# rohitsinghlab/SAME

Measured on AMD Instinct MI355X. Metric: cell-pairs/sec on 100k×100k cost build + edge-cross sweep; % HBM roofline, higher is better.
Workload: dtype f64

## Files before the change

### include/same_hip_diag.h

```cpp
#ifndef SAME_HIP_DIAG_H
#define SAME_HIP_DIAG_H

#include "same_hip.h"

#ifdef __cplusplus
extern "C" {
#endif

enum { SAME_STAT_LAUNCHES = 0, SAME_STAT_FILLS = 1, SAME_STAT_COPIES = 2, SAME_STAT_WAITS = 3, SAME_STAT_GREEDY_READBACKS = 4, SAME_STAT_COUNT = 5 };
int same_ctx_stat(same_ctx *ctx, int which, int64_t *out);


int same_timer_start(same_ctx *ctx);
int same_timer_stop(same_ctx *ctx, float *out_ms);
int same_timer_mark(same_ctx *ctx);
int same_timer_read(same_ctx *ctx, float *out_ms);

int same_ctx_pci_bus_id(same_ctx *ctx, char *out, size_t out_len);
int same_dev_mem_info(same_ctx *ctx, int64_t *out_free, int64_t *out_total);

#define SAME_SPREAD_INFO_LEN 14
int same_dev_alloc_spread(same_ctx *ctx, size_t bytes, void **out_dptr, int64_t *out_info);

#define SAME_Q32_MAX_TYPES 32
int same_quantize_u32_dev(same_ctx *ctx, const double *dsrc, int64_t n, double offset, double scale,
                          uint32_t *ddst);
int same_dense_cost_q32_dev(same_ctx *ctx, const uint32_t *dAq, const uint32_t *dRq, const double *dA,
                            const double *dR, int T, const double *daxy, const double *drxy, int64_t n_r,
                            int64_t row_begin, int64_t row_end, double w, double inv_scale,
                            double rel_tol, double *dout, int64_t ld);

int same_comm_gather_time(same_ctx *ctx, float *out_ms, int64_t *out_send_bytes);

#ifdef __cplusplus
}
#endif
#endif
```

### same_amd/_lib.py

```python
import ctypes
import os
import sys
import threading

import numpy as np

_HERE = os.path.dirname(os.path.abspath(__file__))
LIB_PATH = os.environ.get("SAME_HIP_LIB") or os.path.join(_HERE, "libsame_hip.so")

c_i64 = ctypes.c_int64
c_int = ctypes.c_int
c_dbl = ctypes.c_double
c_flt = ctypes.c_float
c_vp = ctypes.c_void_p
c_sz = ctypes.c_size_t

UNIQUE_ID_BYTES = 128
ABI_VERSION = 9
DT_U8, DT_I32, DT_U64, DT_F64 = 0, 1, 2, 3
OP_SUM, OP_MAX, OP_MIN = 0, 1, 2
SPREAD_INFO_LEN = 14
MAX_KNN = 448
ALIGN_MAX_KNN = 64
ALIGN_MATCH, ALIGN_DECIDED = 1, 2
MAX_TYPES = 4096

_PROTOTYPES = {
    "same_abi_version": [],
    "same_device_count": [ctypes.POINTER(c_int)],
    "same_ctx_create": [c_int, ctypes.POINTER(c_vp)],
    "same_ctx_destroy": [c_vp],
    "same_ctx_sync": [c_vp],
    "same_strerror": [c_int],
    "same_last_error": [c_vp],
    "same_ctx_info": [c_vp, ctypes.c_char_p, c_sz, ctypes.POINTER(c_int), ctypes.POINTER(c_i64)],
    "same_ctx_pci_bus_id": [c_vp, ctypes.c_char_p, c_sz],
    "same_ctx_stat": [c_vp, c_int, ctypes.POINTER(c_i64)],
    "same_dev_alloc": [c_vp, c_sz, ctypes.POINTER(c_vp)],
    "same_dev_free": [c_vp, c_vp],
    "same_dev_alloc_spread": [c_vp, c_sz, ctypes.POINTER(c_vp), ctypes.POINTER(c_i64)],
    "same_h2d": [c_vp, c_vp, c_vp, c_sz],
    "same_d2h": [c_vp, c_vp, c_vp, c_sz],
    "same_dev_memset": [c_vp, c_vp, c_int, c_sz],
    "same_d2d": [c_vp, c_vp, c_vp, c_sz],
    "same_dev_mem_info": [c_vp, ctypes.POINTER(c_i64), ctypes.POINTER(c_i64)],
    "same_ctx_release_scratch": [c_vp],
    "same_timer_start": [c_vp],
    "same_timer_stop": [c_vp, ctypes.POINTER(c_flt)],
    "same_timer_mark": [c_vp],
    "same_timer_read": [c_vp, ctypes.POINTER(c_flt)],
    "same_pair_cost_f64": [c_vp, c_vp, c_vp, c_i64, c_i64, c_int, c_vp, c_vp, c_vp, c_i64, c_dbl, c_vp],
    "same_pair_cost_f32": [c_vp, c_vp, c_vp, c_i64, c_i64, c_int, c_vp, c_vp, c_vp, c_i64, c_flt, c_vp],
    "same_dense_cost_f64_dev": [c_vp, c_vp, c_vp, c_int, c_vp, c_vp, c_i64, c_i64, c_i64, c_dbl, c_vp, c_i64],
    "same_dense_cost_f32_dev": [c_vp, c_vp, c_vp, c_int, c_vp, c_vp, c_i64, c_i64, c_i64, c_flt, c_vp, c_i64],
    "same_dense_cost_f64": [c_vp, c_vp, c_vp, c_i64, c_i64, c_int, c_vp, c_vp, c_i64, c_i64, c_dbl, c_vp, c_i64],
    "same_dense_cost_f32": [c_vp, c_vp, c_vp, c_i64, c_i64, c_int, c_vp, c_vp, c_i64, c_i64, c_flt, c_vp, c_i64],
    "same_quantize_u32_dev": [c_vp, c_vp, c_i64, c_dbl, c_dbl, c_vp],
    "same_dense_cost_q32_dev": [c_vp, c_vp, c_vp, c_vp, c_vp, c_int, c_vp, c_vp, c_i64, c_i64, c_i64, c_dbl, c_dbl, c_dbl, c_vp, c_i64],
    "same_knn_prune": [c_vp, c_vp, c_i64, c_vp, c_i64, c_i64, c_i64, c_dbl, c_int, c_vp, c_vp, c_vp],
    "same_knn_prune_dev": [c_vp, c_vp, c_vp, c_i64, c_i64, c_i64, c_dbl, c_int, c_vp, c_vp, c_vp],
    "same_knn_index_build": [c_vp, c_vp, c_i64, c_dbl, ctypes.POINTER(c_vp)],
    "same_knn_index_destroy": [c_vp],
    "same_knn_prune_indexed_dev": [c_vp, c_vp, c_vp, c_i64, c_i64, c_int, c_vp, c_vp, c_vp],
    "same_padded_cost_f64_dev": [c_vp, c_vp, c_vp, c_int, c_vp, c_vp, c_i64, c_i64, c_int, c_vp, c_dbl, c_vp],
    "same_padded_cost_f32_dev": [c_vp, c_vp, c_vp, c_int, c_vp, c_vp, c_i64, c_i64, c_int, c_vp, c_flt, c_vp],
    "same_tri_classify": [c_vp, c_vp, c_i64, c_vp, c_i64, c_dbl, c_int, c_dbl, c_vp, c_vp, c_vp, c_vp],
    "same_tri_sign_weight": [c_vp, c_vp, c_vp, c_i64, c_vp, c_i64, c_vp, c_vp],
    "same_sweep_bind": [c_vp, c_vp, c_i64, c_vp, c_vp, c_i64, c_i64, c_vp, c_i64, ctypes.POINTER(c_vp)],
    "same_sweep_unbind": [c_vp],
    "same_orient_sweep": [c_vp, c_vp, c_i64, ctypes.POINTER(c_i64), c_vp, ctypes.POINTER(c_i64), c_vp],
# ... 329 lines not shown
```

### same_amd/csrc/common.h

```cpp
#pragma once
#include <hip/hip_runtime.h>

#include <cstdint>
#include <cstdio>
#include <cstring>
#include <string>
#include <vector>

#include "same_hip_diag.h"

struct ncclComm;

enum Slot {
    SL_A = 0, SL_R, SL_AXY, SL_RXY, SL_PAIRS, SL_OUT0, SL_OUT1, SL_OUT2, SL_TRIS, SL_MATCH,
    SL_SIGN, SL_SIZE, SL_TYPE, SL_FLAG0, SL_FLAG1, SL_FLAG2, SL_COUNTS, SL_X, SL_MASK,
    SL_K_HIST, SL_K_RANK, SL_K_SXY, SL_K_SIDX, SL_K_BBOX, SL_K_START,
    SL_Q_START, SL_Q_RANK, SL_Q_SXY, SL_Q_SIDX,
    SL_COUNT
};

struct same_spread_alloc {
    char *va = nullptr;
    size_t bytes = 0;
    std::vector<void *> handles;
};
void same_spread_release(same_spread_alloc &a);

struct same_ctx {
    int device = -1;
    hipStream_t stream = nullptr;
    hipStream_t comm_stream = nullptr;
    hipEvent_t ev0 = nullptr, ev1 = nullptr;
    hipEvent_t ev_ready = nullptr, ev_gathered = nullptr;
    hipEvent_t ev_gather0 = nullptr;
    bool gather_open = false, gather_stamped = false, in_group = false;
    size_t gather_bytes = 0;
    void *slot[SL_COUNT] = {};
    size_t slot_bytes[SL_COUNT] = {};
    void *pinned = nullptr;
    size_t pinned_bytes = 0;
    std::string err;
    int cu_count = 0;
    ncclComm *comm = nullptr;
    int nranks = 1, rank = 0;
    std::vector<same_spread_alloc> spread;
    int64_t stats[SAME_STAT_COUNT] = {};
};

#define SAME_LAUNCH(ctx, kernel, grid, block, lds, ...)                                  \
    do {                                                                                 \
// ... 123 lines not shown
            csr[2 * (size_t)q] = (int32_t)i;
            csr[2 * (size_t)q + 1] = j;
            out->ccsr[(size_t)q] = costs[p];
        }
    return SAME_OK;
}

int same_pair_rowmin_core(same_ctx *ctx, const int32_t *dpairs, const double *dcosts, int64_t P, int64_t n_m, double *dout);
int same_greedy_core(same_ctx *ctx, const int32_t *dpairs, const double *dcosts, int64_t P, int64_t n_m, int64_t n_r,
                     const uint8_t *dprefer, int32_t *dmatch_pair, int *out_rounds);

constexpr int SAME_GREEDY_BATCH_MAX = 64;
struct same_greedy_state {
    uint8_t *alive = nullptr;
    uint8_t *used = nullptr;
    unsigned long long *key[2] = {nullptr, nullptr};
    unsigned *idx[2] = {nullptr, nullptr};
    unsigned long long *sel = nullptr;
    bool float_costs = false;
};
int same_greedy_rounds_core(same_ctx *ctx, const int32_t *dpairs, const double *dcosts, int64_t P, const unsigned long long *dP,
                            int64_t n_m, int64_t n_r, const same_greedy_state &st, int32_t *dmatch_pair, int first, int count);

constexpr int SAME_LAUNCH_WINDOWS = 8;
struct same_greedy_job {
    const int32_t *pairs = nullptr;
    const double *costs = nullptr;
    int64_t P = 0, n_m = 0, n_r = 0;
    same_greedy_state st;
    int32_t *match_pair = nullptr;
};
int same_greedy_rounds_batch_core(same_ctx *ctx, const same_greedy_job *jobs, int n_jobs, int first, int count);

int same_sort_u64_core(same_ctx *ctx, unsigned long long *dkey, int64_t n_pad);
int same_merge_dedup_core(same_ctx *ctx, const uint8_t *dviol, unsigned viol_mask, const int32_t *dwin, const int32_t *da, const int32_t *dr,
                          int64_t n, int32_t *dout, unsigned long long *dtotal);

struct same_knn_index;
struct same_knn_window_job {
    const int32_t *rows_m = nullptr;
    const unsigned long long *dn_m = nullptr;
    int64_t cap_m = 0;
    const int32_t *rows_r = nullptr;
    const unsigned long long *dn_r = nullptr;
    double box[4] = {0, 0, 0, 0};
    int32_t *idx = nullptr, *cnt = nullptr;
};
int same_knn_window_batch_core(same_ctx *ctx, const same_knn_index *ix, const double *dmov_xy, const same_knn_window_job *jobs, int n_jobs, int k);
struct same_cost_window_job {
    const int32_t *rows = nullptr;
    const unsigned long long *dn = nullptr;
    int64_t cap = 0;
    const int32_t *idx = nullptr;
    void *out = nullptr;
};
int same_padded_cost_window_batch_core(same_ctx *ctx, int cost_f32, const void *dA, const void *dR, int T, const void *daxy_c, const void *drxy_c,
                                       const same_cost_window_job *jobs, int n_jobs, int k, double w);
```

### same_amd/csrc/merge.hip

```cpp
#include <algorithm>

#include "common.h"
#include "scan.h"

namespace {

constexpr int SORT_BLOCK = 2048;

__global__ __launch_bounds__(256) void merge_key_kernel(const uint8_t *__restrict__ viol, unsigned viol_mask, const int32_t *__restrict__ window, int64_t n,
                                                          int64_t n_pad, unsigned long long *__restrict__ key) {
    const int64_t i = (int64_t)blockIdx.x * blockDim.x + threadIdx.x;
    if (i >= n_pad) return;
    key[i] = i < n ? ((unsigned long long)((viol[i] & viol_mask) ? 1 : 0) << 63) | ((unsigned long long)(uint32_t)window[i] << 32) | (unsigned long long)i
                   : ~0ull;
}

__global__ __launch_bounds__(256) void bitonic_global_kernel(unsigned long long *__restrict__ key, int64_t n_pad, int64_t j, int64_t k) {
    const int64_t t = (int64_t)blockIdx.x * blockDim.x + threadIdx.x;
    if (t >= n_pad / 2) return;
    const int64_t lo = ((t / j) * 2 * j) + (t % j), hi = lo + j;
    const bool up = (lo & k) == 0;
    const unsigned long long a = key[lo], b = key[hi];
    if ((a > b) == up) { key[lo] = b; key[hi] = a; }
}

__global__ __launch_bounds__(1024) void bitonic_lds_kernel(unsigned long long *__restrict__ key, int64_t k, int j_top) {
    __shared__ unsigned long long s[SORT_BLOCK];
    const int64_t base = (int64_t)blockIdx.x * SORT_BLOCK;
    s[threadIdx.x] = key[base + threadIdx.x];
    s[threadIdx.x + 1024] = key[base + threadIdx.x + 1024];
    __syncthreads();
    for (int j = j_top; j >= 1; j >>= 1) {
        const int t = threadIdx.x;
        const int lo = ((t / j) * 2 * j) + (t % j), hi = lo + j;
        const bool up = ((base + lo) & k) == 0;
        const unsigned long long a = s[lo], b = s[hi];
        if ((a > b) == up) { s[lo] = b; s[hi] = a; }
        __syncthreads();
    }
    key[base + threadIdx.x] = s[threadIdx.x];
    key[base + threadIdx.x + 1024] = s[threadIdx.x + 1024];
}

__global__ __launch_bounds__(1024) void bitonic_lds_head_kernel(unsigned long long *__restrict__ key) {
    __shared__ unsigned long long s[SORT_BLOCK];
    const int64_t base = (int64_t)blockIdx.x * SORT_BLOCK;
    s[threadIdx.x] = key[base + threadIdx.x];
    s[threadIdx.x + 1024] = key[base + threadIdx.x + 1024];
    __syncthreads();
    for (int k = 2; k <= SORT_BLOCK; k <<= 1)
        for (int j = k >> 1; j >= 1; j >>= 1) {
            const int t = threadIdx.x;
            const int lo = ((t / j) * 2 * j) + (t % j), hi = lo + j;
            const bool up = ((base + lo) & k) == 0;
            const unsigned long long a = s[lo], b = s[hi];
            if ((a > b) == up) { s[lo] = b; s[hi] = a; }
            __syncthreads();
        }
    key[base + threadIdx.x] = s[threadIdx.x];
    key[base + threadIdx.x + 1024] = s[threadIdx.x + 1024];
}

__device__ __forceinline__ uint64_t mix64(uint64_t x) {
    x ^= x >> 30; x *= 0xbf58476d1ce4e5b9ull;
    x ^= x >> 27; x *= 0x94d049bb133111ebull;
    return x ^ (x >> 31);
}

constexpr unsigned long long EMPTY = ~0ull;

__device__ __forceinline__ int64_t pair_slot(unsigned long long *__restrict__ tkey, int64_t mask, unsigned long long pair) {
    int64_t h = (int64_t)(mix64(pair) & (uint64_t)mask);
    for (;;) {
        const unsigned long long seen = atomicCAS(&tkey[h], EMPTY, pair);
        if (seen == EMPTY || seen == pair) return h;
        h = (h + 1) & mask;
    }
}

__global__ __launch_bounds__(256) void merge_first_kernel(const unsigned long long *__restrict__ key, int64_t n, const int32_t *__restrict__ a_code,
                                                            const int32_t *__restrict__ r_code, unsigned long long *__restrict__ tkey,
                                                            unsigned int *__restrict__ tfirst, int64_t mask) {
    const int64_t s = (int64_t)blockIdx.x * blockDim.x + threadIdx.x;
    if (s >= n) return;
    const uint32_t row = (uint32_t)key[s];
    const unsigned long long pair = ((unsigned long long)(uint32_t)a_code[row] << 32) | (uint32_t)r_code[row];
    atomicMin(&tfirst[pair_slot(tkey, mask, pair)], (unsigned int)s);
}

__global__ __launch_bounds__(scan::NT) void merge_compact_kernel(const unsigned long long *__restrict__ key, int64_t n, const int32_t *__restrict__ a_code,
                                                                  const int32_t *__restrict__ r_code, unsigned long long *__restrict__ tkey,
                                                                  const unsigned int *__restrict__ tfirst, int64_t mask,
                                                                  unsigned long long *__restrict__ status, int32_t *__restrict__ out_rows,
                                                                  unsigned long long *__restrict__ out_total) {
    __shared__ scan::Shared sh;
    auto keep_of = [&](int64_t q) -> bool {
        if (q >= n) return false;
        const uint32_t row = (uint32_t)key[q];
        const unsigned long long pair = ((unsigned long long)(uint32_t)a_code[row] << 32) | (uint32_t)r_code[row];
        return tfirst[pair_slot(tkey, mask, pair)] == (unsigned int)q;
    };
    const int64_t s0 = (int64_t)blockIdx.x * scan::NT + threadIdx.x;
    const bool keep = keep_of(s0);
    auto val = [&](int64_t q) { return scan::Pair{(q == s0 ? keep : keep_of(q)) ? 1u : 0u, 0u}; };
    scan::Pair through;
    const scan::Pair off = scan::exclusive(status, (int)blockIdx.x, val, sh, &through);
    if (keep) out_rows[off.a] = (int32_t)(uint32_t)key[s0];
    if (blockIdx.x == gridDim.x - 1 && threadIdx.x == 0) *out_total = through.a;
}

}

int same_sort_u64_core(same_ctx *ctx, unsigned long long *dkey, int64_t n_pad) {
    REQUIRE(ctx, n_pad >= SORT_BLOCK && (n_pad & (n_pad - 1)) == 0);
    hipLaunchKernelGGL(bitonic_lds_head_kernel, dim3((unsigned)(n_pad / SORT_BLOCK)), dim3(1024), 0, ctx->stream, dkey);
    for (int64_t k = 2 * SORT_BLOCK; k <= n_pad; k <<= 1) {
        for (int64_t j = k >> 1; j >= SORT_BLOCK; j >>= 1)
            hipLaunchKernelGGL(bitonic_global_kernel, dim3((unsigned)ceil_div(n_pad / 2, 256)), dim3(256), 0, ctx->stream, dkey, n_pad, j, k);
        hipLaunchKernelGGL(bitonic_lds_kernel, dim3((unsigned)(n_pad / SORT_BLOCK)), dim3(1024), 0, ctx->stream, dkey, k, SORT_BLOCK / 2);
    }
    HIP_TRY(ctx, hipGetLastError());
    return SAME_OK;
}

int same_merge_dedup_core(same_ctx *ctx, const uint8_t *dviol, unsigned viol_mask, const int32_t *dwin, const int32_t *da, const int32_t *dr,
                          int64_t n, int32_t *dout, unsigned long long *dtotal) {
    REQUIRE(ctx, n > 0 && n < ((int64_t)1 << 30));
    int64_t n_pad = SORT_BLOCK;
    while (n_pad < n) n_pad <<= 1;
    int64_t slots = 2;
    while (slots < 2 * n) slots <<= 1;
    unsigned long long *dkey, *dtkey, *dstatus;
    unsigned int *dtfirst;
    const size_t st_words = scan::status_bytes(n) / 8;
    SAME_TRY(slot_as(ctx, SL_X, (size_t)n_pad, &dkey));
    SAME_TRY(slot_as(ctx, SL_OUT0, (size_t)slots, &dtkey));
    SAME_TRY(slot_as(ctx, SL_OUT1, (size_t)slots, &dtfirst));
    SAME_TRY(slot_as(ctx, SL_MASK, st_words, &dstatus));
    SAME_FILL(ctx, dtkey, 0xFF, (size_t)slots * 8);
    SAME_FILL(ctx, dtfirst, 0xFF, (size_t)slots * 4);
    SAME_FILL(ctx, dstatus, 0, st_words * 8);
    SAME_LAUNCH(ctx, merge_key_kernel, dim3((unsigned)ceil_div(n_pad, 256)), dim3(256), 0, dviol, viol_mask, dwin, n, n_pad, dkey);
    SAME_TRY(same_sort_u64_core(ctx, dkey, n_pad));
    const unsigned grid = (unsigned)ceil_div(n, 256);
    SAME_LAUNCH(ctx, merge_first_kernel, dim3(grid), dim3(256), 0, dkey, n, da, dr, dtkey, dtfirst, slots - 1);
    SAME_LAUNCH(ctx, merge_compact_kernel, dim3(scan::blocks_for(n)), dim3(scan::NT), 0, dkey, n, da, dr, dtkey, dtfirst, slots - 1,
                scan::arg(dstatus), dout, dtotal);
    HIP_TRY(ctx, hipGetLastError());
    return SAME_OK;
}

extern "C" int same_merge_dedup(same_ctx *ctx, const uint8_t *viol, const int32_t *window_id, const int32_t *aligned_code,
                                const int32_t *ref_code, int64_t n, int32_t *out_rows, int64_t *out_n) {
    REQUIRE(ctx, ctx && out_n && n >= 0 && n < ((int64_t)1 << 30));
    *out_n = 0;
    if (n == 0) return SAME_OK;
    REQUIRE(ctx, viol && window_id && aligned_code && ref_code && out_rows);
    for (int64_t i = 0; i < n; ++i)
        if (window_id[i] < 0 || aligned_code[i] < 0 || ref_code[i] < 0) {
            ctx->err = "same_merge_dedup: window ids and id codes must be non-negative";
            return SAME_ERANGE;
        }
    SAME_TRY(same_use(ctx));
    uint8_t *dviol;
    int32_t *dwin, *da, *dr, *dout;
    unsigned long long *dtotal;
    SAME_TRY(up_as(ctx, SL_FLAG0, viol, (size_t)n, &dviol));
    SAME_TRY(up_as(ctx, SL_PAIRS, window_id, (size_t)n, &dwin));
    SAME_TRY(up_as(ctx, SL_MATCH, aligned_code, (size_t)n, &da));
    SAME_TRY(up_as(ctx, SL_TRIS, ref_code, (size_t)n, &dr));
    SAME_TRY(slot_as(ctx, SL_OUT2, (size_t)n + 4, &dout));
    dtotal = reinterpret_cast<unsigned long long *>(dout + (((size_t)n + 1) & ~size_t(1)));
    SAME_TRY(same_merge_dedup_core(ctx, dviol, 0xFFu, dwin, da, dr, n, dout, dtotal));
    unsigned long long total = 0;
    SAME_TRY(same_down(ctx, &total, dtotal, sizeof total));
    HIP_TRY(ctx, hipStreamSynchronize(ctx->stream));
    REQUIRE(ctx, (int64_t)total <= n);
    SAME_TRY(same_down(ctx, out_rows, dout, (size_t)total * sizeof(int32_t)));
    HIP_TRY(ctx, hipStreamSynchronize(ctx->stream));
    *out_n = (int64_t)total;
    return SAME_OK;
}
```

### same_amd/csrc/section.hip

```cpp
#include "window_internal.h"

namespace {

using namespace devmath;
using namespace win;

__device__ __forceinline__ int cell_of(double v, double origin, double width, int n) {
    const double f = __builtin_floor((v - origin) / width);
    int c = f < 0.0 ? 0 : (f >= (double)n ? n - 1 : (int)f);
    while (c > 0 && v < cell_edge(origin, width, c)) --c;
    while (c < n - 1 && v >= cell_edge(origin, width, c + 1)) ++c;
    return c;
}

__global__ __launch_bounds__(256) void bin_key_kernel(const double *__restrict__ xy, int64_t n, int64_t n_pad, BinGrid g,
                                                       unsigned long long *__restrict__ key) {
    const int64_t i = (int64_t)blockIdx.x * blockDim.x + threadIdx.x;
    if (i >= n_pad) return;
    unsigned long long k = ~0ull;
    if (i < n) {
        const double2_t p = ld2(xy, i);
        if (p.x - p.x == 0.0 && p.y - p.y == 0.0) {
            const int cx = cell_of(p.x, g.x0, g.cw, g.nx), cy = cell_of(p.y, g.y0, g.ch, g.ny);
            k = ((unsigned long long)((unsigned)cy * (unsigned)g.nx + (unsigned)cx) << 32) | (unsigned long long)i;
// ... 32 lines not shown
    for (int off = 32; off > 0; off >>= 1) {
        const unsigned long long a = __shfl_xor(kx0, off, 64), b = __shfl_xor(ky0, off, 64), c = __shfl_xor(kx1, off, 64),
                                 d = __shfl_xor(ky1, off, 64);
        kx0 = a < kx0 ? a : kx0; ky0 = b < ky0 ? b : ky0; kx1 = c > kx1 ? c : kx1; ky1 = d > ky1 ? d : ky1;
    }
    if ((threadIdx.x & 63) == 0) {
        atomicMin(&bbox[0], kx0); atomicMin(&bbox[1], ky0); atomicMax(&bbox[2], kx1); atomicMax(&bbox[3], ky1);
    }
}
double host_key_to_double(unsigned long long k) {
    const unsigned long long u = (k >> 63) ? (k & 0x7FFFFFFFFFFFFFFFull) : ~k;
    double d;
    memcpy(&d, &u, sizeof d);
    return d;
}

__global__ __launch_bounds__(256) void to_float_kernel(const double *__restrict__ src, int64_t n, float *__restrict__ dst) {
    const int64_t i = (int64_t)blockIdx.x * blockDim.x + threadIdx.x;
    if (i < n) dst[i] = (float)src[i];
}

int bin_section(same_ctx *ctx, same_section *s, double x0, double y0, double cw, double ch, bool default_grid) {
    const int64_t n = s->n;
    BinGrid g;
    std::vector<unsigned> h_starts;
    int32_t *order = nullptr;
    unsigned *starts = nullptr;
    int64_t n_binned = 0;
    if (n > 0) {
        unsigned long long *dbbox = nullptr, hb[4] = {~0ull, ~0ull, 0ull, 0ull};
        HIP_TRY(ctx, hipMalloc(reinterpret_cast<void **>(&dbbox), sizeof hb));
        hipError_t e = hipMemcpyAsync(dbbox, hb, sizeof hb, hipMemcpyHostToDevice, ctx->stream);
        if (e == hipSuccess) {
            hipLaunchKernelGGL(bin_bbox_kernel, dim3((unsigned)std::min<int64_t>(ceil_div(n, 256), 256)), dim3(256), 0, ctx->stream, s->xy, n, dbbox);
            e = hipMemcpyAsync(hb, dbbox, sizeof hb, hipMemcpyDeviceToHost, ctx->stream);
        }
        if (e == hipSuccess) e = hipStreamSynchronize(ctx->stream);
        (void)hipFree(dbbox);
        if (e != hipSuccess) return same_fail(ctx, SAME_EIO, "section bounding box", e);
        const bool any = hb[0] != ~0ull;
        if (any) {
            const double mx0 = host_key_to_double(hb[0]), my0 = host_key_to_double(hb[1]), mx1 = host_key_to_double(hb[2]),
                         my1 = host_key_to_double(hb[3]);
            if (default_grid) {
                const double side = std::sqrt((double)n / 512.0);
                const int want = (int)std::min(128.0, std::max(1.0, std::floor(side)));
                x0 = mx0; y0 = my0;
                cw = (mx1 - mx0) / want; ch = (my1 - my0) / want;
                if (!(cw > 0.0) || !std::isfinite(cw)) cw = 1.0;
                if (!(ch > 0.0) || !std::isfinite(ch)) ch = 1.0;
            }
            auto fit = [](double origin, double width, double lo, double hi, double *o_out, int *n_out) -> bool {
                double shift = origin > lo ? std::ceil((origin - lo) / width) : 0.0;
                if (!(shift < 1e9)) return false;
                double o = origin - shift * width;
                while (o > lo) { shift += 1.0; o = origin - shift * width; }
                double cells = std::floor((hi - o) / width) + 1.0;
                if (!(cells < 1e9)) return false;
                int nn = (int)std::max(1.0, cells);
                while (!(cell_edge(o, width, nn) > hi)) {
                    if (nn >= (1 << 30)) return false;
                    ++nn;
                }
                *o_out = o;
                *n_out = nn;
                return true;
            };
            REQUIRE(ctx, fit(x0, cw, mx0, mx1, &g.x0, &g.nx) && fit(y0, ch, my0, my1, &g.y0, &g.ny));
            g.cw = cw;
            g.ch = ch;
            REQUIRE(ctx, (int64_t)g.nx * g.ny <= MAX_GRID_CELLS);
        }
        const int64_t cells = (int64_t)g.nx * g.ny;
        int64_t n_pad = 2048;
        while (n_pad < n) n_pad <<= 1;
        unsigned long long *key = nullptr;
        HIP_TRY(ctx, hipMalloc(reinterpret_cast<void **>(&key), (size_t)n_pad * 8));
        int rc = SAME_OK;
        e = hipMalloc(reinterpret_cast<void **>(&order), (size_t)n * sizeof(int32_t));
        if (e == hipSuccess) e = hipMalloc(reinterpret_cast<void **>(&starts), (size_t)(cells + 1) * sizeof(unsigned));
        if (e == hipSuccess) {
            hipLaunchKernelGGL(bin_key_kernel, dim3(grid_for(n_pad)), dim3(256), 0, ctx->stream, s->xy, n, n_pad, g, key);
            rc = same_sort_u64_core(ctx, key, n_pad);
            if (rc == SAME_OK) {
                hipLaunchKernelGGL(bin_order_kernel, dim3(grid_for(n)), dim3(256), 0, ctx->stream, key, n, order);
                hipLaunchKernelGGL(bin_starts_kernel, dim3(grid_for(cells + 1)), dim3(256), 0, ctx->stream, key, n, cells, starts);
                h_starts.resize((size_t)cells + 1);
                e = hipGetLastError();
                if (e == hipSuccess) e = hipMemcpyAsync(h_starts.data(), starts, (size_t)(cells + 1) * sizeof(unsigned), hipMemcpyDeviceToHost, ctx->stream);
                if (e == hipSuccess) e = hipStreamSynchronize(ctx->stream);
            }
        }
        (void)hipFree(key);
        if (e != hipSuccess || rc != SAME_OK) {
            if (order) (void)hipFree(order);
            if (starts) (void)hipFree(starts);
            return rc != SAME_OK ? rc : same_fail(ctx, e == hipErrorOutOfMemory ? SAME_ENOMEM : SAME_EIO, "section grid", e);
        }
        n_binned = (int64_t)h_starts[(size_t)cells];
    } else {
        h_starts.assign(2, 0u);
    }
    std::unique_lock<std::shared_mutex> swap_hold(s->grid_lock);
    if (s->order || s->starts) (void)hipDeviceSynchronize();
    if (s->order) (void)hipFree(s->order);
    if (s->starts) (void)hipFree(s->starts);
    s->grid = g;
    s->order = order;
    s->starts = starts;
    s->h_starts.swap(h_starts);
    s->n_binned = n_binned;
    ++s->bins;
    return SAME_OK;
}

}

namespace win {

// ... 172 lines not shown
```

### same_amd/csrc/window_internal.h

```cpp
#pragma once
#include <algorithm>
#include <cmath>
#include <memory>
#include <mutex>
#include <new>
#include <shared_mutex>
#include <utility>
#include <vector>

#include "common.h"
#include "devmath.h"
#include "scan.h"
#include "window_state.h"

struct same_knn_index;
extern "C" int same_knn_index_build(same_ctx *ctx, const double *drxy, int64_t n_r, double radius, same_knn_index **out);
extern "C" void same_knn_index_destroy(same_knn_index *ix);

namespace win {

constexpr int MAX_RUN_CELLS = 64;
constexpr int64_t MAX_GRID_CELLS = (int64_t)1 << 22;
constexpr unsigned OUTSIDE = 0x80000000u;

// ... 241 lines not shown
    u.status[1] = cv.scan_words(rows);
    u.totals = cv.take<unsigned long long>(2 * UNPACK_TOTALS);
    u.zero_bytes = cv.off;
    u.pair_off = cv.take<unsigned>((size_t)rows);
    u.work_off = cv.take<unsigned>((size_t)rows);
    u.bytes = cv.off;
}

constexpr int SCORE_TOTALS = 8;
struct ScoreWork {
    int32_t *match_of = nullptr;
    unsigned *node_tri = nullptr, *node_flip = nullptr;
    unsigned long long *totals = nullptr;
    size_t ones_bytes = 0, bytes = 0;
};
inline void lay(ScoreWork &s, Carver &cv, int64_t rows) {
    s.match_of = cv.take<int32_t>((size_t)rows);
    s.ones_bytes = cv.off;
    s.node_tri = cv.take<unsigned>((size_t)rows);
    s.node_flip = cv.take<unsigned>((size_t)rows);
    s.totals = cv.take<unsigned long long>(2 * SCORE_TOTALS);
    s.bytes = cv.off;
}

}

struct same_merge_acc {
    same_ctx *ctx = nullptr;
    int64_t cap = 0;
    int32_t *a_row = nullptr, *r_row = nullptr, *wid = nullptr, *pos = nullptr, *cidx = nullptr;
    uint8_t *flags = nullptr;
    unsigned long long *dcount = nullptr;
    int64_t bound = 0;
    win::DevBuf near_start, near_boxes, scan_words;
    int n_pos = 0, all_seam = 0;
    double reach = 0.0;
    win::DevBuf work, out;
    int32_t *ac = nullptr, *rc = nullptr, *row_of = nullptr;
    unsigned long long *counters = nullptr;
    int64_t n_codes_a = 0;
    int64_t n_rows = 0, n_kept = 0, n_rest = 0, n_final = 0;
    int resolved = 0;
    int final_on_host = 0;
    int merged = 0;
    int loaded = 0;
    int64_t loaded_codes_a = 0, loaded_codes_r = 0;
    std::vector<char> host;
    win::DevBuf score;
    win::ScoreWork sw;
    int64_t score_rows = 0;
    int score_set = 0;
    const same_section *pass_mov = nullptr, *pass_ref = nullptr;
    win::DevBuf unpack, unpack_slices, unpack_pairs;
    win::UnpackWork uw;
    int64_t unpack_rows = 0;
    int unpack_set = 0;
};

struct RestRec {
    int32_t row, ac, rc, wid, pos, cidx;
    uint32_t flags;
};
struct FinalRec {
    int32_t a_row, r_row, cidx, wid, pos;
    uint32_t flags;
};
// ... 102 lines not shown
```

### same_amd/csrc/window_merge.hip

```cpp
#include "window_internal.h"


namespace {

using namespace devmath;
using namespace win;
using scan::Pair;

struct CollectArgs {
    const int32_t *match_row;
    const uint8_t *pflag;
    const int32_t *rows_ua;
    const double *axy;
    int64_t n;
    double tx0, tx1, ty0, ty1;
    int32_t wid, pos;
};

__device__ __forceinline__ bool central(const CollectArgs &w, int64_t c) {
    if (c >= w.n || w.match_row[c] < 0) return false;
    const double2_t p = ld2(w.axy, c);
    return p.x >= w.tx0 && p.x < w.tx1 && p.y >= w.ty0 && p.y < w.ty1;
}

// ... 287 lines not shown
    if (!a) return SAME_ENOMEM;
    a->ctx = ctx;
    *out = a;
    HIP_TRY(ctx, hipMalloc(reinterpret_cast<void **>(&a->dcount), (2 + SAME_LAUNCH_WINDOWS) * sizeof(unsigned long long)));
    HIP_TRY(ctx, hipMemsetAsync(a->dcount, 0, (2 + SAME_LAUNCH_WINDOWS) * sizeof(unsigned long long), ctx->stream));
    HIP_TRY(ctx, hipStreamSynchronize(ctx->stream));
    return SAME_OK;
}

void same_merge_acc_destroy(same_merge_acc *a) {
    if (!a) return;
    (void)hipSetDevice(a->ctx->device);
    (void)hipStreamSynchronize(a->ctx->stream);
    free_rows(a);
    if (a->dcount) (void)hipFree(a->dcount);
    for (DevBuf *b : {&a->near_start, &a->near_boxes, &a->scan_words, &a->work, &a->out, &a->score, &a->unpack, &a->unpack_slices, &a->unpack_pairs}) release(*b);
    delete a;
}

int same_merge_acc_begin(same_merge_acc *a, int64_t expected_rows, int n_pos, const int32_t *near_start, const double *near_boxes, double reach,
                         int all_seam) {
    if (!a) return SAME_EINVAL;
    same_ctx *ctx = a->ctx;
    REQUIRE(ctx, expected_rows >= 0 && expected_rows < ((int64_t)1 << 30) && n_pos >= 0 && reach >= 0.0 && reach - reach == 0.0);
    REQUIRE(ctx, !near_start || n_pos == 0 || near_boxes || near_start[n_pos] == 0);
    if (near_start && n_pos > 0) {
        REQUIRE(ctx, near_start[0] == 0);
        for (int q = 0; q < n_pos; ++q) REQUIRE(ctx, near_start[q + 1] >= near_start[q]);
    }
    SAME_TRY(same_use(ctx));
    a->resolved = 0;
    a->loaded = 0;
    a->bound = 0;
    a->n_rows = a->n_kept = a->n_rest = a->n_final = 0;
    a->n_pos = near_start ? n_pos : 0;
    a->all_seam = all_seam ? 1 : 0;
    a->reach = reach;
    SAME_FILL(ctx, a->dcount, 0, (2 + SAME_LAUNCH_WINDOWS) * sizeof(unsigned long long));
    SAME_TRY(reserve_rows(a, expected_rows, 0));
    if (near_start && n_pos > 0) {
        const int64_t n_boxes = near_start[n_pos];
        SAME_TRY(ensure(ctx, a->near_start, (size_t)(n_pos + 1) * sizeof(int32_t)));
        SAME_TRY(ensure(ctx, a->near_boxes, (size_t)std::max<int64_t>(n_boxes, 1) * 4 * sizeof(double)));
        SAME_COPY(ctx, a->near_start.p, near_start, (size_t)(n_pos + 1) * sizeof(int32_t), hipMemcpyHostToDevice);
        if (n_boxes) SAME_COPY(ctx, a->near_boxes.p, near_boxes, (size_t)n_boxes * 4 * sizeof(double), hipMemcpyHostToDevice);
        SAME_WAIT(ctx);
    }
    return SAME_OK;
}

int same_merge_acc_load(same_merge_acc *a, const int32_t *a_code, const int32_t *r_code, const uint8_t *flags, const int32_t *window_ids,
                        const int32_t *pos, const int32_t *cidx, int64_t n, int64_t n_codes_a, int64_t n_codes_r) {
    if (!a) return SAME_EINVAL;
    same_ctx *ctx = a->ctx;
    REQUIRE(ctx, n >= 0 && n < ((int64_t)1 << 30) && n_codes_a >= 0 && n_codes_r >= 0 && n_codes_a < ((int64_t)1 << 31) && n_codes_r < ((int64_t)1 << 31));
    REQUIRE(ctx, n == 0 || (a_code && r_code && flags && window_ids && pos && cidx));
    SAME_TRY(check_index_range(ctx, a_code, n, 0, std::max<int64_t>(n_codes_a, 1), "aligned codes"));
    SAME_TRY(check_index_range(ctx, r_code, n, 0, std::max<int64_t>(n_codes_r, 1), "reference codes"));
    SAME_TRY(check_index_range(ctx, window_ids, n, 0, (int64_t)1 << 31, "window ids"));
    SAME_TRY(same_use(ctx));
    a->resolved = 0;
    a->n_rows = a->n_kept = a->n_rest = a->n_final = 0;
    a->n_pos = 0;
    a->all_seam = 0;
    a->reach = 0.0;
    SAME_TRY(reserve_rows(a, n, 0));
    a->bound = n;
    a->loaded = 1;
    a->loaded_codes_a = n_codes_a;
    a->loaded_codes_r = n_codes_r;
    const unsigned long long cnt[2] = {(unsigned long long)n, 0ull};
    SAME_COPY(ctx, a->dcount, cnt, sizeof cnt, hipMemcpyHostToDevice);
    if (n) {
        int32_t *const dst[5] = {a->a_row, a->r_row, a->wid, a->pos, a->cidx};
        const int32_t *const src[5] = {a_code, r_code, window_ids, pos, cidx};
        for (int f = 0; f < 5; ++f) SAME_COPY(ctx, dst[f], src[f], (size_t)n * sizeof(int32_t), hipMemcpyHostToDevice);
        SAME_COPY(ctx, a->flags, flags, (size_t)n, hipMemcpyHostToDevice);
    }
    SAME_WAIT(ctx);
    return SAME_OK;
}

int same_window_collect(same_window *const *windows, int n_windows, same_merge_acc *a, const double *trims, const int32_t *window_ids,
                        const int32_t *plan_pos) {
    same_ctx *ctx = nullptr;
    SAME_TRY(check_batch(windows, n_windows, &ctx));
    REQUIRE(ctx, a && a->ctx == ctx && trims && window_ids && plan_pos && !a->resolved);
    int64_t add = 0;
    for (int i = 0; i < n_windows; ++i) {
        REQUIRE(ctx, windows[i]->has_results() && window_ids[i] >= 0);
        add += windows[i]->cur.n_ua;
    }
    REQUIRE(ctx, a->bound + add < ((int64_t)1 << 30));
    SAME_TRY(same_use(ctx));
    if (a->bound + add > a->cap) {
        unsigned long long have = 0;
        HIP_TRY(ctx, hipMemcpyAsync(&have, a->dcount, sizeof have, hipMemcpyDeviceToHost, ctx->stream));
        HIP_TRY(ctx, hipStreamSynchronize(ctx->stream));
        SAME_TRY(reserve_rows(a, a->bound + add, (int64_t)have));
    }
    a->bound += add;
    int64_t most = 0;
    for (int i = 0; i < n_windows; ++i) most = std::max(most, windows[i]->cur.n_ua);
    const int64_t stride = (int64_t)(scan::status_bytes(most) / 8);
    SAME_TRY(ensure(ctx, a->scan_words, (size_t)stride * 8 * SAME_LAUNCH_WINDOWS));
    unsigned long long *words = static_cast<unsigned long long *>(a->scan_words.p);
    for (int g = 0; g < n_windows; g += SAME_LAUNCH_WINDOWS) {
        Batch<CollectArgs> b{};
        int n_g = 0;
        int64_t most_g = 0;
        for (int i = g; i < n_windows && i < g + SAME_LAUNCH_WINDOWS; ++i) {
            const same_window *w = windows[i];
            if (w->cur.n_ua == 0) continue;
            const double *t = trims + 4 * i;
            b.w[n_g++] = CollectArgs{w->match_row, w->pflag, w->cur.rows_ua, w->cur.axy_c, w->cur.n_ua, t[0], t[1], t[2], t[3], window_ids[i], plan_pos[i]};
            most_g = std::max(most_g, w->cur.n_ua);
        }
        if (!n_g) continue;
        const dim3 grid(scan::blocks_for(most_g), (unsigned)n_g);
        SAME_LAUNCH(ctx, collect_count_kernel, grid, dim3(scan::NT), 0, b, a->dcount + 2, words, stride);
        SAME_LAUNCH(ctx, collect_write_kernel, grid, dim3(scan::NT), 0, b, a->dcount, scan::arg(words), stride, rows_of(a), a->cap);
        SAME_LAUNCH(ctx, collect_bump_kernel, dim3(1), dim3(1), 0, a->dcount, n_g);
    }
    HIP_TRY(ctx, hipGetLastError());
    return SAME_OK;
}

int same_merge_acc_resolve(same_merge_acc *const *accs, int n_accs, const same_section *mov, const same_section *ref, int64_t *out_counts) {
    if (!accs || n_accs < 1 || !accs[0]) return SAME_EINVAL;
    same_merge_acc *a = accs[0];
    same_ctx *ctx = a->ctx;
    REQUIRE(ctx, n_accs <= 64 && out_counts);
    const bool loaded = a->loaded != 0;
    REQUIRE(ctx, loaded ? (n_accs == 1 && !mov && !ref) : (mov && ref && mov->ctx->device == ctx->device && ref->ctx->device == ctx->device));
    for (int q = 0; q < n_accs; ++q) {
        REQUIRE(ctx, accs[q] && accs[q]->ctx->device == ctx->device && !accs[q]->resolved);
        for (int p = 0; p < q; ++p) REQUIRE(ctx, accs[p] != accs[q]);
    }
    for (int q = 0; q < 4; ++q) out_counts[q] = 0;
    SAME_TRY(same_use(ctx));
    int64_t n = 0;
    SAME_TRY(lay_end_to_end(accs, n_accs, &n));
    for (int q = 0; q < n_accs; ++q) accs[q]->resolved = 1;
    a->n_rows = n;
    a->pass_mov = loaded ? nullptr : mov;
    a->pass_ref = loaded ? nullptr : ref;
    a->n_codes_a = loaded ? a->loaded_codes_a : (mov->id_codes ? mov->n_codes : mov->n);
    const int64_t n_codes_a = std::max<int64_t>(a->n_codes_a, 1),
                  n_codes_r = std::max<int64_t>(loaded ? a->loaded_codes_r : (ref->id_codes ? ref->n_codes : ref->n), 1);
    const int32_t *codes_a = loaded ? nullptr : mov->id_codes, *codes_r = loaded ? nullptr : ref->id_codes;
    const int64_t nn = std::max<int64_t>(n, 1);
    unsigned long long *status, *counters;
    unsigned *deg_a, *deg_r;
    int32_t *kept;
    uint8_t *cls;
    size_t zero_bytes = 0;
    auto lay = [&](Carver cv) {
        status = cv.scan_words(nn);
        counters = cv.take<unsigned long long>(8);
        deg_a = cv.take<unsigned>((size_t)n_codes_a);
        deg_r = cv.take<unsigned>((size_t)n_codes_r);
        zero_bytes = cv.off;
        a->row_of = cv.take<int32_t>((size_t)n_codes_a);
        a->ac = cv.take<int32_t>((size_t)nn);
        a->rc = cv.take<int32_t>((size_t)nn);
        kept = cv.take<int32_t>((size_t)nn);
        cls = cv.take<uint8_t>((size_t)nn);
        return cv.off;
    };
    SAME_TRY(ensure(ctx, a->work, lay(Carver())));
    lay(Carver(a->work.p));
    SAME_FILL(ctx, a->work.p, 0, zero_bytes);
    SAME_FILL(ctx, a->row_of, 0xFF, (size_t)n_codes_a * 4);
    a->counters = counters;
    SAME_TRY(ensure(ctx, a->out, (size_t)nn * sizeof(RestRec)));
    RestRec *rest = static_cast<RestRec *>(a->out.p);
    if (n) {
        SAME_LAUNCH(ctx, codes_kernel, dim3(grid_for(n)), dim3(256), 0, a->a_row, a->r_row, n, codes_a, codes_r, a->ac, a->rc);
        SAME_TRY(same_merge_dedup_core(ctx, a->flags, 1u, a->wid, a->ac, a->rc, n, kept, counters));
        SAME_LAUNCH(ctx, degree_kernel, dim3(grid_for(n)), dim3(256), 0, kept, counters, n, a->ac, a->rc, deg_a, deg_r);
        const SeamArgs seams{a->n_pos ? static_cast<const int32_t *>(a->near_start.p) : nullptr, static_cast<const double *>(a->near_boxes.p),
                             loaded ? nullptr : mov->xy, loaded ? nullptr : ref->xy, a->n_pos, a->all_seam, a->reach};
        SAME_LAUNCH(ctx, classify_kernel, dim3(grid_for(n)), dim3(256), 0, kept, counters, n, a->ac, a->rc, deg_a, deg_r, a->a_row, a->r_row, a->pos,
                    seams, cls, a->row_of);
        SAME_LAUNCH(ctx, rest_kernel, dim3(scan::blocks_for(n)), dim3(scan::NT), 0, kept, counters, cls, a->ac, a->rc, rows_of(a), scan::arg(status), rest,
                    counters + 1);
        HIP_TRY(ctx, hipGetLastError());
        unsigned long long hc[2] = {0, 0};
        SAME_COPY(ctx, hc, counters, sizeof hc, hipMemcpyDeviceToHost);
        SAME_WAIT(ctx);
        REQUIRE(ctx, (int64_t)hc[0] <= n && (int64_t)hc[1] <= (int64_t)hc[0]);
        a->n_kept = (int64_t)hc[0];
        a->n_rest = (int64_t)hc[1];
    }
    a->host.resize((size_t)a->n_rest * sizeof(RestRec) + 64);
    if (a->n_rest) {
        SAME_COPY(ctx, a->host.data(), rest, (size_t)a->n_rest * sizeof(RestRec), hipMemcpyDeviceToHost);
        SAME_WAIT(ctx);
    }
    out_counts[0] = a->n_rows;
    out_counts[1] = a->n_kept;
    out_counts[2] = a->n_rest;
    out_counts[3] = a->n_kept - a->n_rest;
    return SAME_OK;
}

int same_merge_acc_plain(same_merge_acc *const *accs, int n_accs, int64_t *out_n_rows) {
    if (!accs || n_accs < 1 || !accs[0]) return SAME_EINVAL;
    same_merge_acc *a = accs[0];
    same_ctx *ctx = a->ctx;
    REQUIRE(ctx, n_accs <= 64 && out_n_rows && !a->loaded);
    for (int q = 0; q < n_accs; ++q) {
// ... 137 lines not shown
```

Measured before the change: 627.4 billion.

## Replace bitonic sort with masked-bit LSD radix sort on key high word

Replaces the multi-launch bitonic sort of 64-bit keys with an LSD radix sort that only sorts the bits actually in use in the key's high word: viol bit plus window-id bits for merge dedup, cell bits for spatial binning. Each pass runs a histogram, a decoupled-lookback scan and a stable wave-ranked scatter, with a final copy back when the pass count is odd. This removes the O(log^2 n) global bitonic passes and the padding to a power of two, in exchange for a twin buffer and correctness that depends on the low 32 bits (index) already being ordered, which the stable sort preserves. Host code now tracks the maximum window id to size the mask.

```diff
diff --git a/include/same_hip_diag.h b/include/same_hip_diag.h
--- a/include/same_hip_diag.h
+++ b/include/same_hip_diag.h
@@ -9,6 +9,7 @@
 
 enum { SAME_STAT_LAUNCHES = 0, SAME_STAT_FILLS = 1, SAME_STAT_COPIES = 2, SAME_STAT_WAITS = 3, SAME_STAT_GREEDY_READBACKS = 4, SAME_STAT_COUNT = 5 };
 int same_ctx_stat(same_ctx *ctx, int which, int64_t *out);
+int same_merge_dedup_launches(int32_t max_window_id);
 
 
 int same_timer_start(same_ctx *ctx);
diff --git a/same_amd/_lib.py b/same_amd/_lib.py
--- a/same_amd/_lib.py
+++ b/same_amd/_lib.py
@@ -36,6 +36,7 @@
     "same_ctx_info": [c_vp, ctypes.c_char_p, c_sz, ctypes.POINTER(c_int), ctypes.POINTER(c_i64)],
     "same_ctx_pci_bus_id": [c_vp, ctypes.c_char_p, c_sz],
     "same_ctx_stat": [c_vp, c_int, ctypes.POINTER(c_i64)],
+    "same_merge_dedup_launches": [ctypes.c_int32],
     "same_dev_alloc": [c_vp, c_sz, ctypes.POINTER(c_vp)],
     "same_dev_free": [c_vp, c_vp],
     "same_dev_alloc_spread": [c_vp, c_sz, ctypes.POINTER(c_vp), ctypes.POINTER(c_i64)],
diff --git a/same_amd/csrc/common.h b/same_amd/csrc/common.h
--- a/same_amd/csrc/common.h
+++ b/same_amd/csrc/common.h
@@ -16,6 +16,7 @@
     SL_SIGN, SL_SIZE, SL_TYPE, SL_FLAG0, SL_FLAG1, SL_FLAG2, SL_COUNTS, SL_X, SL_MASK,
     SL_K_HIST, SL_K_RANK, SL_K_SXY, SL_K_SIDX, SL_K_BBOX, SL_K_START,
     SL_Q_START, SL_Q_RANK, SL_Q_SXY, SL_Q_SIDX,
+    SL_SORT_TWIN, SL_SORT_WORK,
     SL_COUNT
 };
 
@@ -205,9 +206,22 @@
 };
 int same_greedy_rounds_batch_core(same_ctx *ctx, const same_greedy_job *jobs, int n_jobs, int first, int count);
 
-int same_sort_u64_core(same_ctx *ctx, unsigned long long *dkey, int64_t n_pad);
-int same_merge_dedup_core(same_ctx *ctx, const uint8_t *dviol, unsigned viol_mask, const int32_t *dwin, const int32_t *da, const int32_t *dr,
-                          int64_t n, int32_t *dout, unsigned long long *dtotal);
+constexpr int SAME_SORT_LAUNCHES_PER_PASS = 3;
+inline int same_sort_passes(uint32_t hi_mask) { return (__builtin_popcount(hi_mask) + 7) / 8; }
+inline int same_sort_launches(uint32_t hi_mask) {
+    const int passes = same_sort_passes(hi_mask);
+    return SAME_SORT_LAUNCHES_PER_PASS * passes + (passes & 1);
+}
+inline uint32_t same_bits_of(uint32_t v) {
+    uint32_t m = 0;
+    while (m < v) m = (m << 1) | 1u;
+    return m;
+}
+int same_sort_u64_core(same_ctx *ctx, unsigned long long *dkey, int64_t n, int64_t n_pad, uint32_t hi_mask);
+constexpr int SAME_MERGE_DEDUP_OWN_LAUNCHES = 3;
+inline uint32_t same_merge_hi_mask(int32_t max_win) { return 0x80000000u | same_bits_of((uint32_t)max_win); }
+int same_merge_dedup_core(same_ctx *ctx, const uint8_t *dviol, unsigned viol_mask, const int32_t *dwin, int32_t max_win, const int32_t *da,
+                          const int32_t *dr, int64_t n, int32_t *dout, unsigned long long *dtotal);
 
 struct same_knn_index;
 struct same_knn_window_job {
diff --git a/same_amd/csrc/merge.hip b/same_amd/csrc/merge.hip
--- a/same_amd/csrc/merge.hip
+++ b/same_amd/csrc/merge.hip
@@ -15,50 +15,85 @@
                    : ~0ull;
 }
 
-__global__ __launch_bounds__(256) void bitonic_global_kernel(unsigned long long *__restrict__ key, int64_t n_pad, int64_t j, int64_t k) {
-    const int64_t t = (int64_t)blockIdx.x * blockDim.x + threadIdx.x;
-    if (t >= n_pad / 2) return;
-    const int64_t lo = ((t / j) * 2 * j) + (t % j), hi = lo + j;
-    const bool up = (lo & k) == 0;
-    const unsigned long long a = key[lo], b = key[hi];
-    if ((a > b) == up) { key[lo] = b; key[hi] = a; }
-}
-
-__global__ __launch_bounds__(1024) void bitonic_lds_kernel(unsigned long long *__restrict__ key, int64_t k, int j_top) {
-    __shared__ unsigned long long s[SORT_BLOCK];
-    const int64_t base = (int64_t)blockIdx.x * SORT_BLOCK;
-    s[threadIdx.x] = key[base + threadIdx.x];
-    s[threadIdx.x + 1024] = key[base + threadIdx.x + 1024];
+constexpr int RADIX_DIGITS = 256, RADIX_ROUNDS = 8, RADIX_TILE = scan::NT * RADIX_ROUNDS;
+static_assert(RADIX_DIGITS == scan::NT, "one thread per digit");
+
+__device__ __forceinline__ unsigned digit_of(unsigned long long key, unsigned pass_mask) {
+    const unsigned hi = (unsigned)(key >> 32);
+    unsigned d = 0, at = 0;
+    for (unsigned m = pass_mask; m; m &= m - 1) d |= ((hi >> __builtin_ctz(m)) & 1u) << at++;
+    return d;
+}
+
+__global__ __launch_bounds__(scan::NT) void radix_hist_kernel(const unsigned long long *__restrict__ key, int64_t n, unsigned pass_mask, int digits,
+                                                               int64_t tiles, unsigned *__restrict__ table) {
+    __shared__ unsigned h[RADIX_DIGITS];
+    h[threadIdx.x] = 0u;
     __syncthreads();
-    for (int j = j_top; j >= 1; j >>= 1) {
-        const int t = threadIdx.x;
-        const int lo = ((t / j) * 2 * j) + (t % j), hi = lo + j;
-        const bool up = ((base + lo) & k) == 0;
-        const unsigned long long a = s[lo], b = s[hi];
-        if ((a > b) == up) { s[lo] = b; s[hi] = a; }
+    const int64_t base = (int64_t)blockIdx.x * RADIX_TILE;
+    for (int r = 0; r < RADIX_ROUNDS; ++r) {
+        const int64_t i = base + r * scan::NT + threadIdx.x;
+        if (i < n) atomicAdd(&h[digit_of(key[i], pass_mask)], 1u);
+    }
+    __syncthreads();
+    if ((int)threadIdx.x < digits) table[(int64_t)threadIdx.x * tiles + blockIdx.x] = h[threadIdx.x];
+}
+
+__global__ __launch_bounds__(scan::NT) void radix_scan_kernel(const unsigned *__restrict__ table, int64_t entries, unsigned long long *__restrict__ status,
+                                                               unsigned *__restrict__ offs) {
+    __shared__ scan::Shared sh;
+    auto val = [&](int64_t q) { return scan::Pair{q < entries ? table[q] : 0u, 0u}; };
+    scan::Pair through;
+    const scan::Pair off = scan::exclusive(status, (int)blockIdx.x, val, sh, &through);
+    const int64_t q = (int64_t)blockIdx.x * scan::NT + threadIdx.x;
+    if (q < entries) offs[q] = off.a;
+}
+
+__global__ __launch_bounds__(scan::NT) void radix_scatter_kernel(const unsigned long long *__restrict__ src, int64_t n, unsigned pass_mask, int digits,
+                                                                  int64_t tiles, const unsigned *__restrict__ offs, unsigned long long *__restrict__ dst) {
+    __shared__ unsigned run[RADIX_DIGITS];
+    __shared__ unsigned wcnt[scan::NT / 64][RADIX_DIGITS];
+    const int tid = threadIdx.x, lane = tid & 63, wave = tid >> 6;
+    run[tid] = tid < digits ? offs[(int64_t)tid * tiles + blockIdx.x] : 0u;
+#pragma unroll
+    for (int w = 0; w < scan::NT / 64; ++w) wcnt[w][tid] = 0u;
+    __syncthreads();
+    const int64_t base = (int64_t)blockIdx.x * RADIX_TILE;
+    for (int r = 0; r < RADIX_ROUNDS; ++r) {
+        const int64_t i = base + r * scan::NT + tid;
+        const bool valid = i < n;
+        const unsigned long long key = valid ? src[i] : 0ull;
+        const unsigned d = valid ? digit_of(key, pass_mask) : 0u;
+        unsigned long long peers = __ballot(valid);
+#pragma unroll
+        for (int b = 0; b < 8; ++b) {
+            const bool bit = (d >> b) & 1u;
+            const unsigned long long bal = __ballot(bit);
+            peers &= bit ? bal : ~bal;
+        }
+        const unsigned rank = (unsigned)__builtin_popcountll(peers & ((1ull << lane) - 1ull));
+        if (valid && rank == 0u) wcnt[wave][d] = (unsigned)__builtin_popcountll(peers);
         __syncthreads();
-    }
-    key[base + threadIdx.x] = s[threadIdx.x];
-    key[base + threadIdx.x + 1024] = s[threadIdx.x + 1024];
-}
-
-__global__ __launch_bounds__(1024) void bitonic_lds_head_kernel(unsigned long long *__restrict__ key) {
-    __shared__ unsigned long long s[SORT_BLOCK];
-    const int64_t base = (int64_t)blockIdx.x * SORT_BLOCK;
-    s[threadIdx.x] = key[base + threadIdx.x];
-    s[threadIdx.x + 1024] = key[base + threadIdx.x + 1024];
-    __syncthreads();
-    for (int k = 2; k <= SORT_BLOCK; k <<= 1)
-        for (int j = k >> 1; j >= 1; j >>= 1) {
-            const int t = threadIdx.x;
-            const int lo = ((t / j) * 2 * j) + (t % j), hi = lo + j;
-            const bool up = ((base + lo) & k) == 0;
-            const unsigned long long a = s[lo], b = s[hi];
-            if ((a > b) == up) { s[lo] = b; s[hi] = a; }
-            __syncthreads();
-        }
-    key[base + threadIdx.x] = s[threadIdx.x];
-    key[base + threadIdx.x + 1024] = s[threadIdx.x + 1024];
+        if (valid) {
+            unsigned at = run[d] + rank;
+            for (int w = 0; w < wave; ++w) at += wcnt[w][d];
+            if ((int64_t)at < n) dst[at] = key;
+        }
+        __syncthreads();
+        unsigned add = 0u;
+#pragma unroll
+        for (int w = 0; w < scan::NT / 64; ++w) {
+            add += wcnt[w][tid];
+            wcnt[w][tid] = 0u;
+        }
+        run[tid] += add;
+        __syncthreads();
+    }
+}
+
+__global__ __launch_bounds__(256) void radix_copy_kernel(const unsigned long long *__restrict__ src, int64_t n, unsigned long long *__restrict__ dst) {
+    const int64_t i = (int64_t)blockIdx.x * blockDim.x + threadIdx.x;
+    if (i < n) dst[i] = src[i];
 }
 
 __device__ __forceinline__ uint64_t mix64(uint64_t x) {
@@ -111,21 +146,37 @@
 
 }
 
-int same_sort_u64_core(same_ctx *ctx, unsigned long long *dkey, int64_t n_pad) {
-    REQUIRE(ctx, n_pad >= SORT_BLOCK && (n_pad & (n_pad - 1)) == 0);
-    hipLaunchKernelGGL(bitonic_lds_head_kernel, dim3((unsigned)(n_pad / SORT_BLOCK)), dim3(1024), 0, ctx->stream, dkey);
-    for (int64_t k = 2 * SORT_BLOCK; k <= n_pad; k <<= 1) {
-        for (int64_t j = k >> 1; j >= SORT_BLOCK; j >>= 1)
-            hipLaunchKernelGGL(bitonic_global_kernel, dim3((unsigned)ceil_div(n_pad / 2, 256)), dim3(256), 0, ctx->stream, dkey, n_pad, j, k);
-        hipLaunchKernelGGL(bitonic_lds_kernel, dim3((unsigned)(n_pad / SORT_BLOCK)), dim3(1024), 0, ctx->stream, dkey, k, SORT_BLOCK / 2);
-    }
+int same_sort_u64_core(same_ctx *ctx, unsigned long long *dkey, int64_t n, int64_t n_pad, uint32_t hi_mask) {
+    REQUIRE(ctx, n_pad >= SORT_BLOCK && (n_pad & (n_pad - 1)) == 0 && n >= 0 && n <= n_pad && n < ((int64_t)1 << 31));
+    const int passes = same_sort_passes(hi_mask);
+    if (n < 2 || passes == 0) return SAME_OK;
+    const int64_t tiles = ceil_div(n, RADIX_TILE);
+    const size_t st_words = scan::status_bytes(RADIX_DIGITS * tiles) / 8, table_len = (size_t)RADIX_DIGITS * (size_t)tiles;
+    unsigned long long *twin, *status;
+    SAME_TRY(slot_as(ctx, SL_SORT_TWIN, (size_t)n, &twin));
+    SAME_TRY(slot_as(ctx, SL_SORT_WORK, (size_t)passes * st_words + table_len, &status));
+    unsigned *table = reinterpret_cast<unsigned *>(status + (size_t)passes * st_words), *offs = table + table_len;
+    SAME_FILL(ctx, status, 0, (size_t)passes * st_words * 8);
+    unsigned long long *src = dkey, *dst = twin;
+    uint32_t left = hi_mask;
+    for (int p = 0; p < passes; ++p, std::swap(src, dst)) {
+        uint32_t pass_mask = 0;
+        int bits = 0;
+        for (; left && bits < 8; ++bits, left &= left - 1) pass_mask |= left & (~left + 1u);
+        const int digits = 1 << bits;
+        const int64_t entries = (int64_t)digits * tiles;
+        SAME_LAUNCH(ctx, radix_hist_kernel, dim3((unsigned)tiles), dim3(scan::NT), 0, src, n, pass_mask, digits, tiles, table);
+        SAME_LAUNCH(ctx, radix_scan_kernel, dim3(scan::blocks_for(entries)), dim3(scan::NT), 0, table, entries, scan::arg(status + (size_t)p * st_words), offs);
+        SAME_LAUNCH(ctx, radix_scatter_kernel, dim3((unsigned)tiles), dim3(scan::NT), 0, src, n, pass_mask, digits, tiles, offs, dst);
+    }
+    if (src != dkey) SAME_LAUNCH(ctx, radix_copy_kernel, dim3((unsigned)ceil_div(n, 256)), dim3(256), 0, src, n, dkey);
     HIP_TRY(ctx, hipGetLastError());
     return SAME_OK;
 }
 
-int same_merge_dedup_core(same_ctx *ctx, const uint8_t *dviol, unsigned viol_mask, const int32_t *dwin, const int32_t *da, const int32_t *dr,
-                          int64_t n, int32_t *dout, unsigned long long *dtotal) {
-    REQUIRE(ctx, n > 0 && n < ((int64_t)1 << 30));
+int same_merge_dedup_core(same_ctx *ctx, const uint8_t *dviol, unsigned viol_mask, const int32_t *dwin, int32_t max_win, const int32_t *da,
+                          const int32_t *dr, int64_t n, int32_t *dout, unsigned long long *dtotal) {
+    REQUIRE(ctx, n > 0 && n < ((int64_t)1 << 30) && max_win >= 0);
     int64_t n_pad = SORT_BLOCK;
     while (n_pad < n) n_pad <<= 1;
     int64_t slots = 2;
@@ -141,7 +192,7 @@
     SAME_FILL(ctx, dtfirst, 0xFF, (size_t)slots * 4);
     SAME_FILL(ctx, dstatus, 0, st_words * 8);
     SAME_LAUNCH(ctx, merge_key_kernel, dim3((unsigned)ceil_div(n_pad, 256)), dim3(256), 0, dviol, viol_mask, dwin, n, n_pad, dkey);
-    SAME_TRY(same_sort_u64_core(ctx, dkey, n_pad));
+    SAME_TRY(same_sort_u64_core(ctx, dkey, n, n_pad, same_merge_hi_mask(max_win)));
     const unsigned grid = (unsigned)ceil_div(n, 256);
     SAME_LAUNCH(ctx, merge_first_kernel, dim3(grid), dim3(256), 0, dkey, n, da, dr, dtkey, dtfirst, slots - 1);
     SAME_LAUNCH(ctx, merge_compact_kernel, dim3(scan::blocks_for(n)), dim3(scan::NT), 0, dkey, n, da, dr, dtkey, dtfirst, slots - 1,
@@ -156,11 +207,14 @@
     *out_n = 0;
     if (n == 0) return SAME_OK;
     REQUIRE(ctx, viol && window_id && aligned_code && ref_code && out_rows);
-    for (int64_t i = 0; i < n; ++i)
+    int32_t max_win = 0;
+    for (int64_t i = 0; i < n; ++i) {
         if (window_id[i] < 0 || aligned_code[i] < 0 || ref_code[i] < 0) {
             ctx->err = "same_merge_dedup: window ids and id codes must be non-negative";
             return SAME_ERANGE;
         }
+        max_win = std::max(max_win, window_id[i]);
+    }
     SAME_TRY(same_use(ctx));
     uint8_t *dviol;
     int32_t *dwin, *da, *dr, *dout;
@@ -171,7 +225,7 @@
     SAME_TRY(up_as(ctx, SL_TRIS, ref_code, (size_t)n, &dr));
     SAME_TRY(slot_as(ctx, SL_OUT2, (size_t)n + 4, &dout));
     dtotal = reinterpret_cast<unsigned long long *>(dout + (((size_t)n + 1) & ~size_t(1)));
-    SAME_TRY(same_merge_dedup_core(ctx, dviol, 0xFFu, dwin, da, dr, n, dout, dtotal));
+    SAME_TRY(same_merge_dedup_core(ctx, dviol, 0xFFu, dwin, max_win, da, dr, n, dout, dtotal));
     unsigned long long total = 0;
     SAME_TRY(same_down(ctx, &total, dtotal, sizeof total));
     HIP_TRY(ctx, hipStreamSynchronize(ctx->stream));
@@ -181,3 +235,7 @@
     *out_n = (int64_t)total;
     return SAME_OK;
 }
+
+extern "C" int same_merge_dedup_launches(int32_t max_window_id) {
+    return SAME_MERGE_DEDUP_OWN_LAUNCHES + same_sort_launches(same_merge_hi_mask(max_window_id < 0 ? 0 : max_window_id));
+}
diff --git a/same_amd/csrc/section.hip b/same_amd/csrc/section.hip
--- a/same_amd/csrc/section.hip
+++ b/same_amd/csrc/section.hip
@@ -88,7 +88,7 @@
         HIP_TRY(ctx, hipMalloc(reinterpret_cast<void **>(&dbbox), sizeof hb));
         hipError_t e = hipMemcpyAsync(dbbox, hb, sizeof hb, hipMemcpyHostToDevice, ctx->stream);
         if (e == hipSuccess) {
-            hipLaunchKernelGGL(bin_bbox_kernel, dim3((unsigned)std::min<int64_t>(ceil_div(n, 256), 256)), dim3(256), 0, ctx->stream, s->xy, n, dbbox);
+            SAME_LAUNCH(ctx, bin_bbox_kernel, dim3((unsigned)std::min<int64_t>(ceil_div(n, 256), 256)), dim3(256), 0, s->xy, n, dbbox);
             e = hipMemcpyAsync(hb, dbbox, sizeof hb, hipMemcpyDeviceToHost, ctx->stream);
         }
         if (e == hipSuccess) e = hipStreamSynchronize(ctx->stream);
@@ -136,11 +136,12 @@
         e = hipMalloc(reinterpret_cast<void **>(&order), (size_t)n * sizeof(int32_t));
         if (e == hipSuccess) e = hipMalloc(reinterpret_cast<void **>(&starts), (size_t)(cells + 1) * sizeof(unsigned));
         if (e == hipSuccess) {
-            hipLaunchKernelGGL(bin_key_kernel, dim3(grid_for(n_pad)), dim3(256), 0, ctx->stream, s->xy, n, n_pad, g, key);
-            rc = same_sort_u64_core(ctx, key, n_pad);
+            SAME_LAUNCH(ctx, bin_key_kernel, dim3(grid_for(n_pad)), dim3(256), 0, s->xy, n, n_pad, g, key);
+            const uint32_t cell_bits = same_bits_of((uint32_t)(cells - 1));
+            rc = same_sort_u64_core(ctx, key, n, n_pad, (cell_bits << 1) | 1u);
             if (rc == SAME_OK) {
-                hipLaunchKernelGGL(bin_order_kernel, dim3(grid_for(n)), dim3(256), 0, ctx->stream, key, n, order);
-                hipLaunchKernelGGL(bin_starts_kernel, dim3(grid_for(cells + 1)), dim3(256), 0, ctx->stream, key, n, cells, starts);
+                SAME_LAUNCH(ctx, bin_order_kernel, dim3(grid_for(n)), dim3(256), 0, key, n, order);
+                SAME_LAUNCH(ctx, bin_starts_kernel, dim3(grid_for(cells + 1)), dim3(256), 0, key, n, cells, starts);
                 h_starts.resize((size_t)cells + 1);
                 e = hipGetLastError();
                 if (e == hipSuccess) e = hipMemcpyAsync(h_starts.data(), starts, (size_t)(cells + 1) * sizeof(unsigned), hipMemcpyDeviceToHost, ctx->stream);
diff --git a/same_amd/csrc/window_internal.h b/same_amd/csrc/window_internal.h
--- a/same_amd/csrc/window_internal.h
+++ b/same_amd/csrc/window_internal.h
@@ -297,6 +297,7 @@
     uint8_t *flags = nullptr;
     unsigned long long *dcount = nullptr;
     int64_t bound = 0;
+    int32_t max_wid = 0;
     win::DevBuf near_start, near_boxes, scan_words;
     int n_pos = 0, all_seam = 0;
     double reach = 0.0;
diff --git a/same_amd/csrc/window_merge.hip b/same_amd/csrc/window_merge.hip
--- a/same_amd/csrc/window_merge.hip
+++ b/same_amd/csrc/window_merge.hip
@@ -343,6 +343,7 @@
     a->resolved = 0;
     a->loaded = 0;
     a->bound = 0;
+    a->max_wid = 0;
     a->n_rows = a->n_kept = a->n_rest = a->n_final = 0;
     a->n_pos = near_start ? n_pos : 0;
     a->all_seam = all_seam ? 1 : 0;
@@ -377,6 +378,8 @@
     a->reach = 0.0;
     SAME_TRY(reserve_rows(a, n, 0));
     a->bound = n;
+    a->max_wid = 0;
+    for (int64_t i = 0; i < n; ++i) a->max_wid = std::max(a->max_wid, window_ids[i]);
     a->loaded = 1;
     a->loaded_codes_a = n_codes_a;
     a->loaded_codes_r = n_codes_r;
@@ -411,6 +414,7 @@
         SAME_TRY(reserve_rows(a, a->bound + add, (int64_t)have));
     }
     a->bound += add;
+    for (int i = 0; i < n_windows; ++i) a->max_wid = std::max(a->max_wid, window_ids[i]);
     int64_t most = 0;
     for (int i = 0; i < n_windows; ++i) most = std::max(most, windows[i]->cur.n_ua);
     const int64_t stride = (int64_t)(scan::status_bytes(most) / 8);
@@ -452,7 +456,11 @@
     SAME_TRY(same_use(ctx));
     int64_t n = 0;
     SAME_TRY(lay_end_to_end(accs, n_accs, &n));
-    for (int q = 0; q < n_accs; ++q) accs[q]->resolved = 1;
+    int32_t max_wid = 0;
+    for (int q = 0; q < n_accs; ++q) {
+        accs[q]->resolved = 1;
+        max_wid = std::max(max_wid, accs[q]->max_wid);
+    }
     a->n_rows = n;
     a->pass_mov = loaded ? nullptr : mov;
     a->pass_ref = loaded ? nullptr : ref;
@@ -488,7 +496,7 @@
     RestRec *rest = static_cast<RestRec *>(a->out.p);
     if (n) {
         SAME_LAUNCH(ctx, codes_kernel, dim3(grid_for(n)), dim3(256), 0, a->a_row, a->r_row, n, codes_a, codes_r, a->ac, a->rc);
-        SAME_TRY(same_merge_dedup_core(ctx, a->flags, 1u, a->wid, a->ac, a->rc, n, kept, counters));
+        SAME_TRY(same_merge_dedup_core(ctx, a->flags, 1u, a->wid, max_wid, a->ac, a->rc, n, kept, counters));
         SAME_LAUNCH(ctx, degree_kernel, dim3(grid_for(n)), dim3(256), 0, kept, counters, n, a->ac, a->rc, deg_a, deg_r);
         const SeamArgs seams{a->n_pos ? static_cast<const int32_t *>(a->near_start.p) : nullptr, static_cast<const double *>(a->near_boxes.p),
                              loaded ? nullptr : mov->xy, loaded ? nullptr : ref->xy, a->n_pos, a->all_seam, a->reach};
```

Measured after the change: 625.6 billion. About the same (-0.3%).
